# sqliteai/sqlite-vector

Hardware: AMD Instinct MI355X
Metric: vectors scanned/sec, L2 top-20 over Nx384 f32 (higher is better)
Workload: dtype f32; 1 GPU; 10Mx384 f32 L2 top-20 single-query; rows_per_gpu=10000000, dim=384, k=20, backend=HIP gfx950 x1

## Files before the change

include/vectorgpu_diag.h:

```cpp
#ifndef VECTORGPU_DIAG_H
#define VECTORGPU_DIAG_H

#include "vectorgpu.h"

#ifdef __cplusplus
extern "C" {
#endif

int vg_set_profiling(vg_corpus *c, int enabled);
int vg_last_kernel_ms(vg_corpus *c, float *scan_ms, float *merge_ms);
int vg_profile_mean_ms(vg_corpus *c, int *n_launches, float *scan_ms, float *merge_ms);
int vg_profile_mean_ms_ex(vg_corpus *c, int *n_launches, float *scan_ms, float *merge_ms, float *prepass_ms);
int vg_plan_scan_shape(int vtype, int dim, int metric, int *lanes_per_row, int *chunks_per_lane, int *long_rows);
int vg_batch_h_plan(long long stride_bytes, int k, int nq, int *waves, int *blocks_per_cu);
const char *vg_scan_kernel_name(vg_corpus *c, int metric);
int vg_filter_exact_evals(vg_corpus *c, unsigned long long *out_evals);
int vg_filter_guard_cooldown(vg_corpus *c);
int vg_batch_filter_exact_evals(vg_corpus *c, unsigned long long *out_evals);
void vg_reload_switches(void);
int vg_batch_last_path(const vg_corpus *c);
int vg_batch_q8_status(const vg_corpus *c);
int vg_batch_masked_plan(const vg_corpus *c, int metric, int *out_queries_per_pass, int *out_lpr, int *out_u);

int vg_corpus_pass_ms(const vg_corpus *c, int which, float *out_ms, long long *out_rows);
long long vg_stat_rows_appended(void);

int vg_shards_gather_stats(vg_shards *s, unsigned long long *out2);
int vg_shards_threaded(const vg_shards *s);
int vg_corpus_tie_stats(const vg_corpus *c, unsigned long long *out4);
int vg_shards_tie_stats(const vg_shards *s, unsigned long long *out4);
int vg_corpus_device_bytes(const vg_corpus *c, long long *out3);
int vg_shards_device_bytes(const vg_shards *s, long long *out3);
int vg_scan_distances_resident(vg_corpus *c, int metric, const void *query);
int vg_resident_distances_fetch(vg_corpus *c, int64_t pos0, int64_t n, float *out_host);
int vg_resident_distances_below(vg_corpus *c, int64_t pos0, float bound, uint64_t *out_pairs, int64_t cap, int64_t *out_count);

int vg_within_set_initial_capacity(vg_corpus *c, int64_t keys);
int vg_within_last_launches(const vg_corpus *c);
int vg_shards_within_set_initial_capacity(vg_shards *s, int64_t keys);
int vg_shards_within_last_launches(const vg_shards *s);

int vg_reference_topk_replay(const float *dist, int64_t n, int k, int64_t below_cap, int64_t *out_pos, double *out_dist);
int vg_reference_topk_replay_slabs(const float *dist, int64_t n, int k, int64_t slab_rows, int64_t below_cap, int64_t *out_pos, double *out_dist);


#ifdef __cplusplus
// ... 4 lines not shown
```

sqlite-vector_amd/__init__.py:

```python
import ctypes as C
import os

import numpy as np

HERE = os.path.dirname(os.path.abspath(__file__))
LIB_PATH = os.environ.get("VG_LIB_PATH") or os.path.join(HERE, "libvectorgpu.so")
EXT_PATH = os.path.join(HERE, "vector.so")

F32, F16, BF16, U8, I8 = 1, 2, 3, 4, 5
L2, SQUARED_L2, COSINE, DOT, L1 = 1, 2, 3, 4, 5
QUANT_U8, QUANT_S8 = 1, 2
TIE_POSITION, TIE_REFERENCE = 0, 1
KEY_EMPTY = 0xFFFFFFFFFFFFFFFF
HALF_TYPES = True
TYPE_SIZE = {F32: 4, F16: 2, BF16: 2, U8: 1, I8: 1}


class VectorGpuError(RuntimeError):
    pass


_lib = None


# ... 48 lines not shown
        "vg_scan_topk_keys": (i32, [vp, i32, vp, i32, vp, C.POINTER(i32)]),
        "vg_scan_topk_enqueue": (i32, [vp, i32, vp, i32]),
        "vg_scan_topk_collect": (i32, [vp, vp]),
        "vg_scan_topk_batch_keys": (i32, [vp, i32, vp, i32, i32, vp, vp]),
        "vg_shards_create": (i32, [vp, i32, i32, i32, i64, C.POINTER(vp)]),
        "vg_shards_destroy": (None, [vp]),
        "vg_shards_clear": (i32, [vp]),
        "vg_shards_count": (i32, [vp]),
        "vg_shards_rows": (i64, [vp]),
        "vg_shards_shard": (vp, [vp, i32]),
        "vg_shards_reserve": (i32, [vp, i64]),
        "vg_shards_set_rowid_base": (i32, [vp, i64]),
        "vg_shards_append": (i32, [vp, vp, i64, i64, vp]),
        "vg_shards_append_records": (i32, [vp, vp, i64]),
        "vg_shards_rowid_at": (i64, [vp, i64]),
        "vg_shards_scan_topk": (i32, [vp, i32, vp, i32, vp, vp, C.POINTER(i32)]),
        "vg_shards_scan_topk_batch": (i32, [vp, i32, vp, i32, i32, vp, vp, vp]),
        "vg_shards_scan_distances": (i32, [vp, i32, vp, vp]),
        "vg_shards_minmax": (i32, [vp, C.POINTER(C.c_float), C.POINTER(C.c_float), C.POINTER(i32)]),
        "vg_shards_quantize_rows": (i32, [vp, C.c_float, C.c_float, i32, i64, i64, vp]),
        "vg_merge_keys_batch": (i32, [vp, i32, i32, i32, vp, i32, vp, vp, vp]),
        "vg_scan_distances": (i32, [vp, i32, vp, vp]),
        "vg_scan_distances_device": (i32, [vp, i32, vp, vp, vp]),
        "vg_corpus_rowid_at": (i64, [vp, i64]),
        "vg_scan_topk_batch": (i32, [vp, i32, vp, i32, i32, vp, vp, vp]),
        "vg_quantize_query": (i32, [i32, vp, i32, C.c_float, C.c_float, i32, vp]),
        "vg_corpus_minmax": (i32, [vp, C.POINTER(C.c_float), C.POINTER(C.c_float), C.POINTER(i32)]),
        "vg_corpus_quantize_rows": (i32, [vp, C.c_float, C.c_float, i32, i64, i64, vp]),
        "vg_set_profiling": (i32, [vp, i32]),
        "vg_last_kernel_ms": (i32, [vp, C.POINTER(C.c_float), C.POINTER(C.c_float)]),
        "vg_profile_mean_ms": (i32, [vp, C.POINTER(i32), C.POINTER(C.c_float), C.POINTER(C.c_float)]),
        "vg_scan_kernel_name": (C.c_char_p, [vp, i32]),
        "vg_plan_scan_shape": (i32, [i32, i32, i32, C.POINTER(i32), C.POINTER(i32), C.POINTER(i32)]),
        "vg_batch_h_plan": (i32, [i64, i32, i32, C.POINTER(i32), C.POINTER(i32)]),
        "vg_profile_mean_ms_ex": (i32, [vp, C.POINTER(i32), C.POINTER(C.c_float), C.POINTER(C.c_float), C.POINTER(C.c_float)]),
        "vg_corpus_find_rowid": (i64, [vp, i64]),
        "vg_corpus_patch_rows": (i32, [vp, vp, i64, vp, i64]),
        "vg_corpus_delete_rows": (i32, [vp, vp, i64]),
        "vg_shards_find_rowid": (i64, [vp, i64]),
        "vg_shards_patch_rows": (i32, [vp, vp, i64, vp, i64]),
        "vg_shards_delete_rows": (i32, [vp, vp, i64]),
        "vg_filter_exact_evals": (i32, [vp, C.POINTER(C.c_ulonglong)]),
        "vg_filter_guard_cooldown": (i32, [vp]),
        "vg_batch_filter_exact_evals": (i32, [vp, C.POINTER(C.c_ulonglong)]),
        "vg_reload_switches": (None, []),
        "vg_batch_last_path": (i32, [vp]),
        "vg_batch_q8_status": (i32, [vp]),
        "vg_corpus_set_scan_filter": (i32, [vp, i32]),
        "vg_corpus_set_tie_order": (i32, [vp, i32]),
        "vg_corpus_tie_order": (i32, [vp]),
        "vg_corpus_tie_stats": (i32, [vp, vp]),
        "vg_corpus_pass_ms": (i32, [vp, i32, C.POINTER(C.c_float), C.POINTER(C.c_longlong)]),
        "vg_shards_set_tie_order": (i32, [vp, i32]),
        "vg_shards_set_scan_filter": (i32, [vp, i32]),
        "vg_shards_set_gather": (i32, [vp, i32]),
        "vg_shards_gather_stats": (i32, [vp, vp]),
        "vg_shards_tie_stats": (i32, [vp, vp]),
        "vg_shards_threaded": (i32, [vp]),
        "vg_slab_scan_begin": (i32, [i32, i32, i32, i32, vp, i32, i32, i64, i64, vp]),
        "vg_slab_scan_rows": (i32, [vp, vp, i64, i64, vp]),
        "vg_slab_scan_records": (i32, [vp, vp, i64]),
        "vg_slab_scan_finish": (i32, [vp, vp, vp, vp]),
        "vg_slab_scan_all": (i32, [vp, vp, vp, vp]),
        "vg_slab_scan_destroy": (None, [vp]),
        "vg_device_memory": (i32, [i32, vp, vp]),
        "vg_host_alloc": (i32, [C.c_size_t, C.POINTER(C.c_void_p)]),
# ... 135 lines not shown
        rows = np.ascontiguousarray(rows)
        assert rows.ndim == 2 and rows.shape[1] * rows.itemsize >= self.dim * TYPE_SIZE[self.vtype]
        ids = None if rowids is None else np.ascontiguousarray(rowids, dtype=np.int64)
        _check(lib().vg_corpus_append(self.h, _ptr(rows), rows.shape[0], rows.strides[0], _ptr(ids)))

    def append_strided(self, buf, n_rows, stride, rowids=None):
        buf = np.ascontiguousarray(buf)
        ids = None if rowids is None else np.ascontiguousarray(rowids, dtype=np.int64)
        _check(lib().vg_corpus_append(self.h, _ptr(buf), n_rows, stride, _ptr(ids)))

    def append_records(self, records, n):
        records = np.ascontiguousarray(records)
        _check(lib().vg_corpus_append_records(self.h, _ptr(records), n))

    def append_device(self, dev_ptr, n_rows, stride, rowids=None):
        ids = None if rowids is None else np.ascontiguousarray(rowids, dtype=np.int64)
        _check(lib().vg_corpus_append_device(self.h, C.c_void_p(dev_ptr), n_rows, stride, _ptr(ids)))

    def set_rowid_base(self, base):
        _check(lib().vg_corpus_set_rowid_base(self.h, base))

    def scan_topk(self, metric, query, k):
        query = np.ascontiguousarray(query)
        ids = np.zeros(max(k, 1), dtype=np.int64)
        dist = np.zeros(max(k, 1), dtype=np.float64)
        cnt = C.c_int(0)
        _check(lib().vg_scan_topk(self.h, metric, _ptr(query), k, _ptr(ids), _ptr(dist), C.byref(cnt)))
        return ids[:cnt.value], dist[:cnt.value]

    def scan_topk_device(self, metric, dev_query_ptr, k, dev_keys_ptr, stream=None):
        _check(lib().vg_scan_topk_device(self.h, metric, C.c_void_p(dev_query_ptr), k, C.c_void_p(dev_keys_ptr),
                                         C.c_void_p(stream) if stream else None))

    def scan_distances(self, metric, query):
        query = np.ascontiguousarray(query)
        out = np.empty(self.rows, dtype=np.float32)
        _check(lib().vg_scan_distances(self.h, metric, _ptr(query), _ptr(out)))
        return out

    def scan_within(self, metric, query, radius, limit=None):
        query = np.ascontiguousarray(query)
        m, held = C.c_int64(0), C.c_int64(0)
        _check(lib().vg_scan_within(self.h, metric, _ptr(query), float(radius), 0 if limit is None else max(int(limit), 0), C.byref(m), C.byref(held)))
        n = 0 if (limit is not None and limit <= 0) else held.value
        ids, dist = np.zeros(n, dtype=np.int64), np.zeros(n, dtype=np.float64)
        if n:
            _check(lib().vg_scan_within_fetch(self.h, 0, n, _ptr(ids), _ptr(dist)))
        return ids, dist, m.value

    def set_mask(self, bits=None, positions=None, rowids=None):
        return _set_mask(self, "vg_corpus", self.rows, bits, positions, rowids)

    def clear_mask(self):
        _check(lib().vg_corpus_clear_mask(self.h))

    def mask_count(self):
        return int(lib().vg_corpus_mask_count(self.h))

    def scan_topk_masked(self, metric, query, k):
        query = np.ascontiguousarray(query)
        ids = np.zeros(max(k, 1), dtype=np.int64)
        dist = np.zeros(max(k, 1), dtype=np.float64)
        cnt = C.c_int(0)
        _check(lib().vg_scan_topk_masked(self.h, metric, _ptr(query), k, _ptr(ids), _ptr(dist), C.byref(cnt)))
        return ids[:cnt.value], dist[:cnt.value]

# ... 392 lines not shown
```

sqlite-vector_amd/csrc/vg_api.hip:

```cpp
#include "vg_internal.h"

#include "vg_scan.h"


typedef void (*scan_fn_t)(ScanArgs);
scan_fn_t vg_pick_scan_kernel_ex(int vtype, int acc, int U);

typedef VgShape Shape;

static const int kAllowedU[] = {1, 2, 3, 4, 6, 8};

static int max_chunks_per_lane(int vtype, int acc, bool bf16_l2_u3) {
    if (vtype == VG_TYPE_F16) return 6;
    if (vtype == VG_TYPE_BF16) return (acc == A_L2 && !bf16_l2_u3) ? 6 : 3;
    return 8;
}

struct ShapeEnv { bool f16_round3, pref_round1, bf16_l2_u3, int_short_round3, force_long; int lpr_log2, u; };
static ShapeEnv shape_env() {
    ShapeEnv e;
    e.f16_round3 = vg_sw(SW_VG_SHAPE_F16_ROUND3, 0) != 0;
    e.pref_round1 = vg_sw(SW_VG_SHAPE_PREF_ROUND1, 0) != 0;
    e.bf16_l2_u3 = vg_sw(SW_VG_SHAPE_BF16_L2_U3, 0) != 0;
    e.int_short_round3 = vg_sw(SW_VG_SHAPE_INT_SHORT_ROUND3, 0) != 0;
// ... 172 lines not shown



#define VG_MERGE_THREADS 1024
__global__ __launch_bounds__(VG_MERGE_THREADS) void vg_merge_kernel(const uint64_t *cand, int nlists, int k,
                                                                    uint64_t *out_keys, const unsigned long long *mirror_src,
                                                                    unsigned long long *mirror_dst) {
    __shared__ __attribute__((aligned(16))) uint8_t scratch[VG_SEL_SCRATCH_BYTES];
    if (mirror_dst && blockIdx.x == 0 && threadIdx.x < 3) mirror_dst[threadIdx.x] = mirror_src[threadIdx.x];
    vg_select_lists(cand + (long long)blockIdx.x * nlists * VG_WAVE, nlists, k, out_keys + (long long)blockIdx.x * VG_WAVE, scratch);
}

int vg_launch_merge(const uint64_t *dev_cand, int nlists, int k, uint64_t *dev_out_keys, int nq, hipStream_t stream) {
    hipLaunchKernelGGL(vg_merge_kernel, dim3((unsigned)nq), dim3(VG_MERGE_THREADS), 0, stream, dev_cand, nlists, k, dev_out_keys,
                       (const unsigned long long *)nullptr, (unsigned long long *)nullptr);
    return (int)hipGetLastError();
}

static int launch_scan(vg_corpus *c, int metric, const uint8_t *dev_query, int k, uint64_t *dev_out_keys,
                       float *dev_out_dist, hipStream_t stream, const ScanPlan &plan = ScanPlan());

int vg_launch_plain_scan(vg_corpus *c, int metric, const uint8_t *dev_query, int k, uint64_t *dev_out_keys, hipStream_t stream,
                         const ScanPlan &plan) {
    return launch_scan(c, metric, dev_query, k, dev_out_keys, nullptr, stream, plan);
}
int vg_launch_merge_one(const uint64_t *dev_cand, int nlists, int k, uint64_t *dev_out_keys, hipStream_t stream,
                        const unsigned long long *mirror_src, unsigned long long *mirror_dst) {
    hipLaunchKernelGGL(vg_merge_kernel, dim3(1), dim3(VG_MERGE_THREADS), 0, stream, dev_cand, nlists, k, dev_out_keys, mirror_src, mirror_dst);
    return (int)hipGetLastError();
}
int vg_plain_scan_shape(const vg_corpus *c, int metric, VgShape *out) {
    choose_shape(c->nch, c->vtype, vg_metric_to_acc(metric), out);
    return 0;
}
long long vg_plain_scan_blocks(const vg_corpus *c, int64_t n_rows, const VgShape &s) {
    const int rpb = VG_WAVE >> s.lpr_log2;
    const long long nbatch = (n_rows + rpb - 1) / rpb;
    const int bpc = std::max(1, std::min(8, vg_sw(SW_VG_BLOCKS_PER_CU, 1)));
    long long blocks = (nbatch + VG_WAVES_PER_BLOCK - 1) / VG_WAVES_PER_BLOCK;
    blocks = std::max<long long>(1, std::min<long long>(blocks, (long long)c->cu_count * bpc));
    blocks = std::min<long long>(blocks, VG_SEL_MAX_HEADS);
    blocks = std::min<long long>(blocks, std::max<long long>(32, nbatch / (2 * VG_WAVES_PER_BLOCK)));
    return blocks;
}

static int launch_scan(vg_corpus *c, int metric, const uint8_t *dev_query, int k, uint64_t *dev_out_keys,
                       float *dev_out_dist, hipStream_t stream, const ScanPlan &plan) {
    int acc = vg_metric_to_acc(metric);
    if (acc < 0) return vg_fail(VG_ERR_INVALID, "unknown distance metric %d", metric);
    const int64_t n_rows = (plan.n_rows >= 0) ? std::min<int64_t>(plan.n_rows, c->n_rows) : c->n_rows;
    if (plan.ref_emit) c->ref_prefix_rows = -1;
    Shape s;
    choose_shape(c->nch, c->vtype, acc, &s);
    const bool whole_prefix = plan.ref_emit && !dev_out_dist && plan.n_rows < 0 && k > 0 && k <= VG_MAX_FUSED_K && !s.long_rows &&
                              n_rows < VG_REF_EMIT_MIN_ROWS;
    if (!whole_prefix && plan.allow_filter && plan.n_rows < 0 && !dev_out_dist && k <= VG_MAX_FUSED_K) {
        int rcf = vg_launch_scan_filter(c, metric, dev_query, k, dev_out_keys, stream, plan.ref_emit, plan.final_out);
        if (rcf != -1) return rcf;
    }
    if (acc == A_COS && (c->vtype == VG_TYPE_F16 || c->vtype == VG_TYPE_BF16) && !s.long_rows && vg_sw(SW_VG_HALF_COSN, 1)) {
        int rcn = vg_ensure_row_norms(c);
        if (rcn != VG_OK) return rcn;
        acc = A_COSN;
        if (stream != c->stream) {
            if (!c->norm_ev) HIP_TRY(hipEventCreateWithFlags(&c->norm_ev, hipEventDisableTiming));
            HIP_TRY(hipEventRecord(c->norm_ev, c->stream));
// ... 7 lines not shown
    if (whole_prefix) {
        int rcb = vg_ensure_ref_buffers(c, n_rows);
        if (rcb != VG_OK) return rcb;
        store_prefix = c->d_ref_prefix;
        emit_reset = c->d_below;
        c->ref_prefix_rows = n_rows;
    }
    const bool prefix_pass = store_prefix && !dev_out_dist && !s.long_rows && k > 0;
    scan_fn_t fn = (emitting || prefix_pass) ? vg_pick_scan_kernel_ex(c->vtype, acc, s.U) : pick_kernel(c->vtype, acc, s, use_nt_loads(c, n_rows));
    if (!fn) return vg_fail(VG_ERR_UNSUPPORTED, "no scan kernel for type %s", type_tag(c->vtype));

    const long long blocks = vg_plain_scan_blocks(c, n_rows, s);

    ScanArgs a{};
    a.rows = c->d_rows;
    a.query = dev_query;
    a.cand = plan.lists_out ? plan.lists_out : c->d_cand;
    a.out_dist = dev_out_dist;
    a.n_rows = n_rows;
    a.stride = c->stride;
    a.nch = c->nch;
    a.lpr_log2 = s.lpr_log2;
    a.k = k;
    a.root = (metric == VG_DIST_L2) ? 1 : 0;
    a.dim = c->dim;
    a.row_nn = (acc == A_COSN) ? c->d_xnorm : nullptr;
    a.init_keys = nullptr;
    a.emit = nullptr;
    a.emit_cap = 0;
    a.emit_reset = emit_reset;
    a.order = scan_order_for(c, n_rows);
    if (prefix_pass) a.out_dist = store_prefix;
    else a.emit_reset = nullptr;
    size_t qbytes = (size_t)c->nch * 16;
    if (s.long_rows) {
        const size_t slice = (size_t)VG_WAVE * VG_LONG_U;
        qbytes = ((c->nch + slice - 1) / slice) * slice * 16;
    }
    size_t smem = std::max<size_t>(qbytes, (size_t)VG_PUBLISH_LDS_BYTES);
    a.store_lds_off = 0;
    if (dev_out_dist && !s.long_rows) {
        a.store_lds_off = (int)((qbytes + 255) / 256 * 256);
        smem = std::max<size_t>(smem, (size_t)a.store_lds_off + (size_t)VG_WAVES_PER_BLOCK * VG_STORE_FLOATS * sizeof(float));
    }

    if (c->append_pending && stream != c->stream) HIP_TRY(hipStreamWaitEvent(stream, c->append_ev, 0));

    hipEvent_t *evs = plan.record ? vg_prof_slot(c, (uint8_t)((dev_out_dist == nullptr ? VG_EVF_MERGE : 0) | (emitting ? VG_EVF_PREPASS : 0))) : nullptr;
    if (evs) hipEventRecord(evs[0], stream);
    if (emitting) {
        const int64_t P = vg_ref_prefix_for(n_rows);
        int rcb = vg_ensure_ref_buffers(c, P);
        if (rcb != VG_OK) return rcb;
        ScanPlan pre;
        pre.n_rows = P;
        pre.allow_filter = false;
        pre.record = false;
        pre.store_prefix = c->d_ref_prefix;
        pre.emit_reset = c->d_below;
        int rcp = launch_scan(c, metric, dev_query, k, dev_out_keys, nullptr, stream, pre);
        if (rcp != VG_OK) return rcp;
        a.init_keys = dev_out_keys;
        a.emit = c->d_below;
        a.emit_cap = VG_BELOW_CAP;
        c->ref_prefix_rows = P;
        if (evs) hipEventRecord(evs[1], stream);
    }
    if (smem > 64 * 1024)
        HIP_TRY(hipFuncSetAttribute(reinterpret_cast<const void *>(fn), hipFuncAttributeMaxDynamicSharedMemorySize, (int)smem));
    hipLaunchKernelGGL(fn, dim3((unsigned)blocks), dim3(VG_BLOCK), smem, stream, a);
    if (evs) hipEventRecord(evs[2], stream);
    if (plan.lists_out) {
        if (plan.n_lists_out) *plan.n_lists_out = (int)blocks;
    } else if (!dev_out_dist) {
        hipLaunchKernelGGL(vg_merge_kernel, dim3(1), dim3(VG_MERGE_THREADS), 0, stream,
                           (const uint64_t *)c->d_cand, (int)blocks, k, plan.final_out ? plan.final_out : dev_out_keys,
                           (const unsigned long long *)nullptr, (unsigned long long *)nullptr);
    }
    if (evs) hipEventRecord(evs[3], stream);
    HIP_TRY(hipGetLastError());
    return VG_OK;
}

static bool host_direct(const vg_corpus *c) {
    const int v = vg_sw(SW_VG_HOST_DIRECT, -1);
    if (v >= 0) return v != 0;
    return c->n_rows * c->stride <= (64ll << 20);
}

static void stage_query(vg_corpus *c, const void *query) {
    memset(c->h_query, 0, (size_t)c->stride);
    memcpy(c->h_query, query, (size_t)c->dim * c->es);
}

static void slot_times(vg_corpus *c, int slot, float *scan_ms, float *merge_ms, float *prepass_ms) {
    hipEvent_t *evs = &c->ev[(size_t)slot * VG_PROF_EVS];
    const uint8_t fl = c->ev_flags[(size_t)slot];
    hipEventSynchronize(evs[3]);
    *scan_ms = 0.f; *merge_ms = 0.f; *prepass_ms = 0.f;
    if (fl & VG_EVF_PREPASS) hipEventElapsedTime(prepass_ms, evs[0], evs[1]);
    hipEventElapsedTime(scan_ms, evs[(fl & VG_EVF_PREPASS) ? 1 : 0], evs[2]);
    if (fl & VG_EVF_MERGE) hipEventElapsedTime(merge_ms, evs[2], evs[3]);
}

void vg_collect_timing(vg_corpus *c) {
    if (!c->profiling || c->prof_launches == 0) return;
    slot_times(c, (int)((c->prof_launches - 1) % VG_PROF_RING), &c->last_scan_ms, &c->last_merge_ms, &c->last_prepass_ms);
}

extern "C" float vg_key_distance(uint64_t key) { return vg_sortable_f32((uint32_t)(key >> 32)); }
extern "C" uint32_t vg_key_position(uint64_t key) { return (uint32_t)(key & 0xFFFFFFFFull); }

extern "C" int vg_scan_topk_device(vg_corpus *c, int metric, const void *dev_query, int k, uint64_t *dev_out_keys,
                                   void *stream) {
    if (!c || !dev_query || !dev_out_keys) return vg_fail(VG_ERR_INVALID, "vg_scan_topk_device: NULL argument");
    if (k < 1 || k > VG_MAX_FUSED_K) return vg_fail(VG_ERR_UNSUPPORTED, "vg_scan_topk_device: k must be in 1..%d", VG_MAX_FUSED_K);
    HIP_TRY(hipSetDevice(c->device));
    hipStream_t st = stream ? (hipStream_t)stream : c->stream;
    if (c->n_rows == 0) {
        HIP_TRY(hipMemsetAsync(dev_out_keys, 0xFF, VG_WAVE * sizeof(uint64_t), st));
        return VG_OK;
    }
    return launch_scan(c, metric, (const uint8_t *)dev_query, k, dev_out_keys, nullptr, st);
}

extern "C" int vg_scan_distances_device(vg_corpus *c, int metric, const void *dev_query, float *dev_out_dist, void *stream) {
    if (!c || !dev_query || !dev_out_dist) return vg_fail(VG_ERR_INVALID, "vg_scan_distances_device: NULL argument");
    HIP_TRY(hipSetDevice(c->device));
    if (c->n_rows == 0) return VG_OK;
    return launch_scan(c, metric, (const uint8_t *)dev_query, 0, nullptr, dev_out_dist, stream ? (hipStream_t)stream : c->stream);
}
// ... 279 lines not shown
```

sqlite-vector_amd/csrc/vg_corpus.hip:

```cpp
#include "vg_internal.h"

#include <atomic>
#include <mutex>
#include <utility>
#include <vector>

#include "vg_device.h"


static thread_local std::string g_err;

int vg_fail(int code, const char *fmt, ...) {
    char buf[1024];
    va_list ap;
    va_start(ap, fmt);
    vsnprintf(buf, sizeof(buf), fmt, ap);
    va_end(ap);
    g_err = buf;
    return code;
}

extern "C" const char *vg_last_error(void) { return g_err.c_str(); }
extern "C" void vg_set_last_error_(const char *msg) { g_err = msg ? msg : ""; }

// ... 36 lines not shown
    {"VG_BATCH_LONG_BPC", 1},
    {"VG_BATCH_MFMA", 0},
    {"VG_BATCH_MIN_QUERIES", 1},
    {"VG_BATCH_PREPASS", 1},
    {"VG_BATCH_Q8", 0},
    {"VG_BATCH_SLICE", 0},
    {"VG_BATCH_STAGES", 0},
    {"VG_BATCH_TILE_MAJOR", 0},
    {"VG_BLOCKS_PER_CU", 1},
    {"VG_F32_FILTER", 0},
    {"VG_FILTER_LPR_LOG2", 1},
    {"VG_FILTER_U", 1},
    {"VG_FORCE_LONG", 0},
    {"VG_HALF_COSN", 1},
    {"VG_HOST_DIRECT", 1},
    {"VG_KEYS_DIRECT", 1},
    {"VG_LPR_LOG2", 1},
    {"VG_MULTI_SCAN", 0},
    {"VG_NT", 1},
    {"VG_Q8_TWO_READS", 1},
    {"VG_RADIX_SELECT", 0},
    {"VG_REF_ALWAYS_EMIT", 1},
    {"VG_REF_STORE_MODE", 0},
    {"VG_SCAN_FILTER", 0},
    {"VG_SCAN_FILTER_MIN_MB", 0},
    {"VG_SCAN_FILTER_MIRROR_COPY", 1},
    {"VG_SCAN_FILTER_N4", 0},
    {"VG_SCAN_FILTER_NO_GUARD", 0},
    {"VG_SCAN_FILTER_PREMERGE", 1},
    {"VG_SCAN_FILTER_PREPASS", 1},
    {"VG_SCAN_FILTER_PREPASS_DIV", 1},
    {"VG_SCAN_FILTER_SHADOW", 0},
    {"VG_SCAN_ORDER", 1},
    {"VG_SHAPE_BF16_L2_U3", 1},
    {"VG_SHAPE_F16_ROUND3", 1},
    {"VG_SHAPE_INT_SHORT_ROUND3", 1},
    {"VG_SHAPE_PREF_ROUND1", 1},
    {"VG_U", 1},
};
std::atomic<int> vg_switch_values[VGSW_COUNT];
void vg_switches_read(void) {
    for (int i = 0; i < VGSW_COUNT; ++i) {
        int v = VGSW_UNSET;
#ifndef VG_LAB
        if (!vg_switch_names[i].lab)
#endif
        {
            const char *e = getenv(vg_switch_names[i].name);
            if (e && *e) {
                if (i == SW_VG_SCAN_FILTER_SHADOW) v = (unsigned char)e[0];
                else if (i == SW_VECTORGPU_SHARD_GATHER) v = (e[0] == 'r' || e[0] == 'R') ? 1 : 0;
                else v = atoi(e);
            }
        }
        vg_switch_values[i].store(v, std::memory_order_relaxed);
    }
}
__attribute__((constructor)) static void vg_switches_at_load(void) { vg_switches_read(); }
extern "C" void vg_reload_switches(void) { vg_switches_read(); }

extern "C" int vg_corpus_create(int device, int vtype, int dim, int64_t capacity_rows_hint, vg_corpus **out) {
    if (!out) return vg_fail(VG_ERR_INVALID, "vg_corpus_create: out is NULL");
    *out = nullptr;
    vg_switches_read();
    int es = vg_elem_size(vtype);
    if (es == 0) return vg_fail(VG_ERR_INVALID, "vg_corpus_create: unknown vector type %d", vtype);
    if (dim <= 0) return vg_fail(VG_ERR_INVALID, "vg_corpus_create: dimension must be positive (got %d)", dim);
    int ndev = vg_device_count();
    if (ndev <= 0) return vg_fail(VG_ERR_NO_DEVICE, "no HIP device available (the scan path is GPU-only)");
    if (device < 0 || device >= ndev) return vg_fail(VG_ERR_INVALID, "device %d out of range (0..%d)", device, ndev - 1);
    int64_t row_bytes = (int64_t)dim * es;
    if (row_bytes > 128 * 1024) return vg_fail(VG_ERR_UNSUPPORTED, "rows larger than 128 KiB are not supported (dim=%d): the query must fit the CU's 160 KiB LDS", dim);
    HIP_TRY(hipSetDevice(device));
    vg_corpus *c = new vg_corpus();
    c->device = device;
    c->vtype = vtype;
    c->dim = dim;
    c->es = es;
    c->nch = (int)((row_bytes + 15) / 16);
    c->stride = (int64_t)c->nch * 16;
    hipDeviceProp_t p;
    if (hipGetDeviceProperties(&p, device) != hipSuccess) { delete c; return vg_fail(VG_ERR_HIP, "hipGetDeviceProperties failed"); }
    c->cu_count = p.multiProcessorCount;
    c->max_blocks = c->cu_count * 8;
    hipError_t e;
    if ((e = hipStreamCreateWithFlags(&c->stream, hipStreamNonBlocking)) != hipSuccess ||
        (e = hipMalloc(&c->d_query, (size_t)c->stride)) != hipSuccess ||
        (e = hipHostMalloc(&c->h_query, (size_t)c->stride)) != hipSuccess ||
        (e = hipMalloc(&c->d_cand, (size_t)c->max_blocks * VG_WAVE * sizeof(uint64_t))) != hipSuccess ||
        (e = hipMalloc(&c->d_keys, VG_WAVE * sizeof(uint64_t))) != hipSuccess ||
        (e = hipHostMalloc(&c->h_keys, VG_WAVE * sizeof(uint64_t))) != hipSuccess) {
        vg_corpus_destroy(c);
        return vg_fail(VG_ERR_HIP, "vg_corpus_create: device setup failed: %s", hipGetErrorString(e));
    }
    if (capacity_rows_hint > 0) {
        e = hipMalloc(&c->d_rows, (size_t)(capacity_rows_hint * c->stride));
        if (e != hipSuccess) {
            vg_corpus_destroy(c);
            return vg_fail(VG_ERR_NOMEM, "vg_corpus_create: cannot allocate %lld bytes of HBM: %s",
                           (long long)(capacity_rows_hint * c->stride), hipGetErrorString(e));
        }
        c->cap_rows = capacity_rows_hint;
    }
    *out = c;
    return VG_OK;
}

extern "C" void vg_corpus_destroy(vg_corpus *c) {
    if (!c) return;
    hipSetDevice(c->device);
    if (c->stream) hipStreamSynchronize(c->stream);
    if (c->d_rows) hipFree(c->d_rows);
    if (c->d_query) hipFree(c->d_query);
    if (c->h_query) hipHostFree(c->h_query);
    if (c->d_cand) hipFree(c->d_cand);
    if (c->d_cand_pre) hipFree(c->d_cand_pre);
    if (c->d_keys) hipFree(c->d_keys);
    if (c->h_keys) hipHostFree(c->h_keys);
    if (c->d_dist) hipFree(c->d_dist);
    if (c->d_sel_keys) hipFree(c->d_sel_keys);
    if (c->d_sel_sorted) hipFree(c->d_sel_sorted);
    if (c->d_sel_temp) hipFree(c->d_sel_temp);
    for (int i = 0; i < 2; ++i) { if (c->pin[i]) hipHostFree(c->pin[i]); if (c->pin_ev[i]) hipEventDestroy(c->pin_ev[i]); }
    if (c->append_ev) hipEventDestroy(c->append_ev);
    if (c->d_stage) hipFree(c->d_stage);
    if (c->d_bq) hipFree(c->d_bq);
    if (c->h_bq) hipHostFree(c->h_bq);
// ... 677 lines not shown
```

sqlite-vector_amd/csrc/vg_device.h:

```cpp
#pragma once

#include <hip/hip_runtime.h>
#include <stdint.h>

#define VG_EMPTY_KEY 0xFFFFFFFFFFFFFFFFull
#define VG_WAVE 64
#define VG_BLOCK 1024
#define VG_WAVES_PER_BLOCK (VG_BLOCK / VG_WAVE)
#define VG_MAX_FUSED_K 64

enum { T_F32 = 1, T_F16 = 2, T_BF16 = 3, T_U8 = 4, T_I8 = 5 };
enum { M_L2 = 1, M_SQL2 = 2, M_COS = 3, M_DOT = 4, M_L1 = 5 };
enum { A_L2 = 0, A_COS = 1, A_DOT = 2, A_L1 = 3, A_COSN = 4  };

struct ScanArgs {
    const uint8_t *rows;
    const uint8_t *query;
    uint64_t *cand;
    float *out_dist;
    long long n_rows;
    long long stride;
    int nch;
    int lpr_log2;
    int k;
    int root;
    int dim;
    const float *row_nn;
    int store_lds_off;
    const uint64_t *init_keys;
    unsigned long long *emit;
    unsigned emit_cap;
    unsigned long long *emit_reset;
    int order;
    float within_r;
    unsigned long long within_cap;
    const uint64_t *mask;
};


__host__ __device__ inline uint32_t vg_f32_sortable(float d) {
    uint32_t b;
#if defined(__HIP_DEVICE_COMPILE__)
    b = __float_as_uint(d);
#else
    __builtin_memcpy(&b, &d, 4);
#endif
    return b ^ ((b >> 31) ? 0xFFFFFFFFu : 0x80000000u);
}
__host__ __device__ inline float vg_sortable_f32(uint32_t s) {
    uint32_t b = s ^ ((s >> 31) ? 0x80000000u : 0xFFFFFFFFu);
#if defined(__HIP_DEVICE_COMPILE__)
    return __uint_as_float(b);
#else
    float f; __builtin_memcpy(&f, &b, 4); return f;
#endif
}
__host__ __device__ inline uint64_t vg_make_key(float d, uint32_t pos) {
    return ((uint64_t)vg_f32_sortable(d) << 32) | (uint64_t)pos;
}


__device__ inline uint64_t vg_readlane64(uint64_t v, int lane_uniform) {
    uint32_t lo = (uint32_t)__builtin_amdgcn_readlane((int)(uint32_t)v, lane_uniform);
    uint32_t hi = (uint32_t)__builtin_amdgcn_readlane((int)(uint32_t)(v >> 32), lane_uniform);
    return ((uint64_t)hi << 32) | lo;
}

__device__ inline uint64_t vg_wave_shr1(uint64_t v) {
    const uint32_t lo = (uint32_t)__builtin_amdgcn_update_dpp(0, (int)(uint32_t)v, 0x138, 0xf, 0xf, false);
// ... 112 lines not shown
```

sqlite-vector_amd/csrc/vg_internal.h:

```cpp
#pragma once

#include "../../include/vectorgpu.h"
#include "../../include/vectorgpu_diag.h"

#include <hip/hip_runtime.h>

#include <algorithm>
#include <cmath>
#include <cstdarg>
#include <cstdio>
#include <cstdlib>
#include <cstring>
#include <string>
#include <vector>

#define VG_PROF_RING 1024
#define VG_PROF_EVS 4
#define VG_EVF_MERGE 1
#define VG_EVF_PREPASS 2
#define VG_WAVE_HOST 64

int vg_fail(int code, const char *fmt, ...);

#define HIP_TRY(expr)                                                                                     \
// ... 2 lines not shown
        if (e__ != hipSuccess)                                                                            \
            return vg_fail(e__ == hipErrorOutOfMemory ? VG_ERR_NOMEM : VG_ERR_HIP, "%s failed: %s (%s:%d)", \
                           #expr, hipGetErrorString(e__), __FILE__, __LINE__);                            \
    } while (0)


static inline int vg_elem_size(int vtype) {
    switch (vtype) {
        case VG_TYPE_F32: return 4;
        case VG_TYPE_F16: case VG_TYPE_BF16: return 2;
        case VG_TYPE_U8: case VG_TYPE_I8: return 1;
    }
    return 0;
}

struct vg_corpus {
    int device = 0;
    int vtype = 0;
    int dim = 0;
    int es = 0;
    int nch = 0;
    int64_t stride = 0;
    int64_t n_rows = 0;
    int64_t cap_rows = 0;
    uint8_t *d_rows = nullptr;
    std::vector<int64_t> rowids;
    bool rowids_ascending = true;
    int64_t rowid_base = 1;

    hipStream_t stream = nullptr;
    uint8_t *d_query = nullptr;
    uint8_t *h_query = nullptr;
    uint64_t *d_cand = nullptr;
    uint64_t *d_cand_pre = nullptr;
    uint64_t *d_keys = nullptr;
    uint64_t *h_keys = nullptr;
    float *d_dist = nullptr;
    int64_t d_dist_cap = 0;
    int64_t dist_valid_rows = 0;
    unsigned long long *d_below = nullptr;
    uint8_t *h_ref = nullptr;
    size_t h_ref_bytes = 0;
    std::vector<uint64_t> ref_pairs;
    int tie_order = 0;
    float *d_ref_prefix = nullptr;
    int64_t ref_prefix_cap = 0;
    int64_t ref_prefix_rows = -1;
    int ref_hot = 0;
    unsigned long long ref_stats[4] = {0, 0, 0, 0};
    uint64_t *d_sel_keys = nullptr, *d_sel_sorted = nullptr;
    void *d_sel_temp = nullptr;
    uint32_t *d_sel_state = nullptr;
    size_t sel_temp_bytes = 0;
    int64_t sel_cap = 0;
    uint8_t *pin[2] = {nullptr, nullptr};
    hipEvent_t pin_ev[2] = {nullptr, nullptr};
    bool pin_busy[2] = {false, false};
    int pin_idx = 0;
    uint8_t *d_stage = nullptr;
    hipEvent_t append_ev = nullptr;
    bool append_pending = false;
    bool enqueued = false;
    float *d_xnorm = nullptr;
    int64_t xnorm_rows = 0, xnorm_cap = 0;
    hipEvent_t norm_ev = nullptr;
    uint32_t *d_sx = nullptr;
// ... 147 lines not shown
```

sqlite-vector_amd/csrc/vg_scan.h:

```cpp
#pragma once

#include "vg_accum.h"
#include "vg_lists.h"

#define VG_PUBLISH_LDS_BYTES (VG_WAVES_PER_BLOCK * VG_WAVE * 8 + VG_SEL_SCRATCH_BYTES)

__device__ inline void vg_block_publish(uint8_t *smem, uint64_t mine, int k, uint64_t *dst) {
    const int lane = threadIdx.x & (VG_WAVE - 1);
    const int wave = threadIdx.x >> 6;
    uint64_t *lists = reinterpret_cast<uint64_t *>(smem);
    lists[wave * VG_WAVE + lane] = (lane < k) ? mine : VG_EMPTY_KEY;
    __syncthreads();
    vg_select_lists(lists, VG_WAVES_PER_BLOCK, k, dst, smem + VG_WAVES_PER_BLOCK * VG_WAVE * 8);
}

typedef uint32_t vg_u32x4 __attribute__((ext_vector_type(4)));

template <bool NT>
__device__ inline uint4 vg_load16(const uint8_t *p) {
    if (NT) {
        vg_u32x4 v = __builtin_nontemporal_load(reinterpret_cast<const vg_u32x4 *>(p));
        return make_uint4(v.x, v.y, v.z, v.w);
    }
    return *reinterpret_cast<const uint4 *>(p);
}

#ifndef VG_LOAD_PREDICATED
#define VG_LOAD_PREDICATED 0
#endif
static __device__ __attribute__((aligned(16))) uint32_t vg_zero_chunk[4] = {0u, 0u, 0u, 0u};

template <int U, bool NT>
__device__ inline void vg_load_batch(uint4 (&dst)[U], const uint8_t *rows, long long row, long long n_rows,
                                     long long stride, int sub, int lpr, int nch) {
    const uint8_t *p = rows + row * stride + (long long)sub * 16;
#pragma unroll
    for (int u = 0; u < U; ++u) {
        const int c = sub + u * lpr;
        if (VG_LOAD_PREDICATED) {
            uint4 v = make_uint4(0u, 0u, 0u, 0u);
            if (row < n_rows && c < nch) v = vg_load16<NT>(p + (long long)u * lpr * 16);
            dst[u] = v;
        } else {
            const uint8_t *src = (row < n_rows && c < nch) ? p + (long long)u * lpr * 16 : reinterpret_cast<const uint8_t *>(vg_zero_chunk);
            dst[u] = vg_load16<NT>(src);
        }
// ... 188 lines not shown
        for (int j = 0; j < NB - 1; ++j) load(buf[j], nn[j], b + j * wstride);
        while (b < b_end) {
#pragma unroll
            for (int j = 0; j < NB; ++j) {
                const long long bj = b + j * wstride;
                load(buf[(j + NB - 1) % NB], nn[(j + NB - 1) % NB], bj + (NB - 1) * wstride);
                if (bj < b_end) process(buf[j], nn[j], bj);
            }
            b += NB * wstride;
        }
    } else {
        load(buf[0], nn[0], b);
        while (b < b_end) {
            const long long bn = b + wstride;
            load(buf[1], nn[1], bn);
            process(buf[0], nn[0], b);
#pragma unroll
            for (int u = 0; u < U; ++u) buf[0][u] = buf[1][u];
            nn[0] = nn[1];
            b = bn;
        }
    }
    if constexpr (WITHIN) {
        if (wqueued > 0) vg_within_flush(wqueue, wqueued, a.emit, a.within_cap, lane);
        return;
    }
    if (store_mode) {
        for (int j = lane; j < in_line * rpb && line_row0 + j < a.n_rows; j += VG_WAVE) a.out_dist[line_row0 + j] = line[j];
        return;
    }

    __syncthreads();
    vg_block_publish(smem, mine, k, a.cand + (long long)blockIdx.x * VG_WAVE);
}

#define VG_LONG_U 2
template <int VT, int ACC, bool NT, bool WITHIN = false, bool MASKED = false>
__global__ __launch_bounds__(VG_BLOCK) void vg_scan_long_kernel(ScanArgs a) {
    extern __shared__ __attribute__((aligned(16))) uint8_t smem[];
    const int lane = threadIdx.x & (VG_WAVE - 1);
    const int wave = threadIdx.x >> 6;
    constexpr int U = VG_LONG_U;
    const int slice = VG_WAVE * U;
    const int S = (a.nch + slice - 1) / slice;
    const int nch_pad = S * slice;

    uint4 *qs = reinterpret_cast<uint4 *>(smem);
    for (int c = threadIdx.x; c < nch_pad; c += VG_BLOCK)
        qs[c] = (c < a.nch) ? reinterpret_cast<const uint4 *>(a.query)[c] : make_uint4(0u, 0u, 0u, 0u);
    __syncthreads();

    typename Accum<VT, ACC>::QStat qstat;
    {
        uint4 q0[U];
#pragma unroll
        for (int u = 0; u < U; ++u) q0[u] = qs[u * VG_WAVE + lane];
        qstat = Accum<VT, ACC>::template query_stat<U>(q0, 6);
        for (int s = 1; s < S; ++s) {
#pragma unroll
            for (int u = 0; u < U; ++u) q0[u] = qs[s * slice + u * VG_WAVE + lane];
            Accum<VT, ACC>::merge_qstat(qstat, Accum<VT, ACC>::template query_stat<U>(q0, 6));
        }
    }

    uint64_t mine = VG_EMPTY_KEY, thr = VG_EMPTY_KEY;
    const int k = a.k;
// ... 41 lines not shown
        if (ns == 0 && (!MASKED || m_cur)) {
            float d = acc.finish(qstat, 6, a.root);
            if constexpr (VT == T_F16 || VT == T_BF16) {
                if (acc.special(qstat, 6) && lane == 0)
                    d = vg_slow_distance<VT, ACC>(reinterpret_cast<const uint16_t *>(qs),
                                                  reinterpret_cast<const uint16_t *>(a.rows + row * a.stride), a.dim, a.root);
            }
            d = vg_clamp(d);
            if constexpr (WITHIN) {
                vg_within_offer(vg_make_key(d, (uint32_t)row), (lane == 0) && (d <= a.within_r) && (d < INFINITY), wqueue, wqueued, a.emit, a.within_cap, lane);
            } else if (store_mode) {
                if (lane == 0) a.out_dist[row] = d;
            } else {
                vg_list_offer(vg_make_key(d, (uint32_t)row), (lane == 0) && (d < INFINITY), mine, thr, lane, k);
            }
            acc.init();
        }
        if constexpr (MASKED) {
            if (ns == 0) { m_cur = m_nxt; m_nxt = vg_mask_bits(a.mask, nrow + wstride, 1, nrow + wstride < a.n_rows) != 0ull; }
        }
#pragma unroll
        for (int u = 0; u < U; ++u) cur[u] = nxt[u];
        row = nrow;
        s = ns;
    }
    if constexpr (WITHIN) {
        if (wqueued > 0) vg_within_flush(wqueue, wqueued, a.emit, a.within_cap, lane);
        return;
    }
    if (store_mode) return;

    __syncthreads();
    vg_block_publish(smem, mine, k, a.cand + (long long)blockIdx.x * VG_WAVE);
}


template <int VT>
__global__ __launch_bounds__(256) void vg_half_rownorm_kernel(const uint8_t *rows, long long row0, long long n, long long stride,
                                                              int nch, float *out) {
    const int sub = threadIdx.x & 15;
    const long long group = ((long long)blockIdx.x * blockDim.x + threadIdx.x) >> 4;
    const long long ngroups = ((long long)gridDim.x * blockDim.x) >> 4;
    for (long long r = group; r < n; r += ngroups) {
        const uint4 *p = reinterpret_cast<const uint4 *>(rows + (row0 + r) * stride);
        double s0 = 0.0, s1 = 0.0, s2 = 0.0, s3 = 0.0;
        for (int c = sub; c < nch; c += 16) {
            const uint4 v = p[c];
            const uint32_t w[4] = {v.x, v.y, v.z, v.w};
#pragma unroll
            for (int j = 0; j < 4; ++j) {
                float lo, hi;
                vg_unpack2<VT>(w[j], lo, hi);
                if (j & 1) { s2 += (double)(lo * lo); s3 += (double)(hi * hi); }
                else { s0 += (double)(lo * lo); s1 += (double)(hi * hi); }
            }
        }
        const double s = vg_group_sum((s0 + s1) + (s2 + s3), 4);
        if (sub == 0) { const float f = (float)s; out[row0 + r] = (s > 0.0 && f == 0.0f) ? 1.401298464324817e-45f : f; }
    }
}
```

sqlite-vector_amd/csrc/vg_switches.h:

```cpp
#pragma once
#include <atomic>
#include <climits>

enum VgSwitch {
    SW_VECTORGPU_SHARD_GATHER,
    SW_VECTORGPU_SHARD_THREADS,
    SW_VG_BATCH_BPC,
    SW_VG_BATCH_H_SPLIT,
    SW_VG_BATCH_H_WAVES,
    SW_VG_BATCH_LONG,
    SW_VG_BATCH_LONG_BPC,
    SW_VG_BATCH_MFMA,
    SW_VG_BATCH_MIN_QUERIES,
    SW_VG_BATCH_PREPASS,
    SW_VG_BATCH_Q8,
    SW_VG_BATCH_SLICE,
    SW_VG_BATCH_STAGES,
    SW_VG_BATCH_TILE_MAJOR,
    SW_VG_BLOCKS_PER_CU,
    SW_VG_F32_FILTER,
    SW_VG_FILTER_LPR_LOG2,
    SW_VG_FILTER_U,
    SW_VG_FORCE_LONG,
    SW_VG_HALF_COSN,
    SW_VG_HOST_DIRECT,
    SW_VG_KEYS_DIRECT,
    SW_VG_LPR_LOG2,
    SW_VG_MULTI_SCAN,
    SW_VG_NT,
    SW_VG_Q8_TWO_READS,
    SW_VG_RADIX_SELECT,
    SW_VG_REF_ALWAYS_EMIT,
    SW_VG_REF_STORE_MODE,
    SW_VG_SCAN_FILTER,
    SW_VG_SCAN_FILTER_MIN_MB,
    SW_VG_SCAN_FILTER_MIRROR_COPY,
    SW_VG_SCAN_FILTER_N4,
    SW_VG_SCAN_FILTER_NO_GUARD,
    SW_VG_SCAN_FILTER_PREMERGE,
    SW_VG_SCAN_FILTER_PREPASS,
    SW_VG_SCAN_FILTER_PREPASS_DIV,
    SW_VG_SCAN_FILTER_SHADOW,
    SW_VG_SCAN_ORDER,
    SW_VG_SHAPE_BF16_L2_U3,
    SW_VG_SHAPE_F16_ROUND3,
    SW_VG_SHAPE_INT_SHORT_ROUND3,
    SW_VG_SHAPE_PREF_ROUND1,
    SW_VG_U,
    VGSW_COUNT
};
#define VGSW_UNSET INT_MIN
extern std::atomic<int> vg_switch_values[VGSW_COUNT];
void vg_switches_read(void);
static inline int vg_sw(VgSwitch id, int dflt) { const int v = vg_switch_values[id].load(std::memory_order_relaxed); return v == VGSW_UNSET ? dflt : v; }
static inline bool vg_sw_set(VgSwitch id) { return vg_switch_values[id].load(std::memory_order_relaxed) != VGSW_UNSET; }
```

Before: 4.425 billion vectors/s.

## Fuse final top-k merge into scan kernel via last-block arrival counter

Adds a device arrival counter so that the last scan block to finish runs the cross-block top-k selection itself and writes the final keys. This removes the separate single-block merge kernel launch and the launch gap that precedes it. The cost is a release/acquire fence plus an atomic per block, and the final merge now runs serialized inside the scan kernel's tail. Profiling events and the candidate buffer allocation are adjusted to match, and a switch lets the path be turned off.

```diff
diff --git a/include/vectorgpu_diag.h b/include/vectorgpu_diag.h
--- a/include/vectorgpu_diag.h
+++ b/include/vectorgpu_diag.h
@@ -12,6 +12,7 @@
 int vg_profile_mean_ms(vg_corpus *c, int *n_launches, float *scan_ms, float *merge_ms);
 int vg_profile_mean_ms_ex(vg_corpus *c, int *n_launches, float *scan_ms, float *merge_ms, float *prepass_ms);
 int vg_plan_scan_shape(int vtype, int dim, int metric, int *lanes_per_row, int *chunks_per_lane, int *long_rows);
+int vg_scan_last_launch(const vg_corpus *c, int *out_blocks, int *out_tail_select);
 int vg_batch_h_plan(long long stride_bytes, int k, int nq, int *waves, int *blocks_per_cu);
 const char *vg_scan_kernel_name(vg_corpus *c, int metric);
 int vg_filter_exact_evals(vg_corpus *c, unsigned long long *out_evals);
diff --git a/sqlite-vector_amd/__init__.py b/sqlite-vector_amd/__init__.py
--- a/sqlite-vector_amd/__init__.py
+++ b/sqlite-vector_amd/__init__.py
@@ -104,6 +104,7 @@
         "vg_profile_mean_ms": (i32, [vp, C.POINTER(i32), C.POINTER(C.c_float), C.POINTER(C.c_float)]),
         "vg_scan_kernel_name": (C.c_char_p, [vp, i32]),
         "vg_plan_scan_shape": (i32, [i32, i32, i32, C.POINTER(i32), C.POINTER(i32), C.POINTER(i32)]),
+        "vg_scan_last_launch": (i32, [vp, C.POINTER(i32), C.POINTER(i32)]),
         "vg_batch_h_plan": (i32, [i64, i32, i32, C.POINTER(i32), C.POINTER(i32)]),
         "vg_profile_mean_ms_ex": (i32, [vp, C.POINTER(i32), C.POINTER(C.c_float), C.POINTER(C.c_float), C.POINTER(C.c_float)]),
         "vg_corpus_find_rowid": (i64, [vp, i64]),
@@ -305,6 +306,11 @@
         _check(lib().vg_scan_topk_device(self.h, metric, C.c_void_p(dev_query_ptr), k, C.c_void_p(dev_keys_ptr),
                                          C.c_void_p(stream) if stream else None))
 
+    def last_scan_launch(self):
+        blocks, tail = C.c_int(0), C.c_int(0)
+        _check(lib().vg_scan_last_launch(self.h, C.byref(blocks), C.byref(tail)))
+        return blocks.value, tail.value
+
     def scan_distances(self, metric, query):
         query = np.ascontiguousarray(query)
         out = np.empty(self.rows, dtype=np.float32)
diff --git a/sqlite-vector_amd/csrc/vg_api.hip b/sqlite-vector_amd/csrc/vg_api.hip
--- a/sqlite-vector_amd/csrc/vg_api.hip
+++ b/sqlite-vector_amd/csrc/vg_api.hip
@@ -228,6 +228,12 @@
 int vg_plain_scan_shape(const vg_corpus *c, int metric, VgShape *out) {
     choose_shape(c->nch, c->vtype, vg_metric_to_acc(metric), out);
     return 0;
+}
+extern "C" int vg_scan_last_launch(const vg_corpus *c, int *out_blocks, int *out_tail_select) {
+    if (!c) return vg_fail(VG_ERR_INVALID, "corpus is NULL");
+    if (out_blocks) *out_blocks = c->last_scan_blocks;
+    if (out_tail_select) *out_tail_select = c->last_scan_tail;
+    return VG_OK;
 }
 long long vg_plain_scan_blocks(const vg_corpus *c, int64_t n_rows, const VgShape &s) {
     const int rpb = VG_WAVE >> s.lpr_log2;
@@ -301,6 +307,13 @@
     a.order = scan_order_for(c, n_rows);
     if (prefix_pass) a.out_dist = store_prefix;
     else a.emit_reset = nullptr;
+    const bool tail = !dev_out_dist && !plan.lists_out && !emitting && !prefix_pass && k >= 1 && c->d_arrive &&
+                      (s.long_rows || vg_tail_fits(c->vtype, acc, s.U)) && vg_sw(SW_VG_SCAN_TAIL_SELECT, 1) != 0;
+    if (tail) {
+        a.final_out = plan.final_out ? plan.final_out : dev_out_keys;
+        a.arrive = c->d_arrive;
+    }
+    if (!dev_out_dist && !plan.lists_out && plan.record) { c->last_scan_blocks = (int)blocks; c->last_scan_tail = tail ? 1 : 0; }
     size_t qbytes = (size_t)c->nch * 16;
     if (s.long_rows) {
         const size_t slice = (size_t)VG_WAVE * VG_LONG_U;
@@ -315,7 +328,7 @@
 
     if (c->append_pending && stream != c->stream) HIP_TRY(hipStreamWaitEvent(stream, c->append_ev, 0));
 
-    hipEvent_t *evs = plan.record ? vg_prof_slot(c, (uint8_t)((dev_out_dist == nullptr ? VG_EVF_MERGE : 0) | (emitting ? VG_EVF_PREPASS : 0))) : nullptr;
+    hipEvent_t *evs = plan.record ? vg_prof_slot(c, (uint8_t)(((dev_out_dist == nullptr && !tail) ? VG_EVF_MERGE : 0) | (emitting ? VG_EVF_PREPASS : 0))) : nullptr;
     if (evs) hipEventRecord(evs[0], stream);
     if (emitting) {
         const int64_t P = vg_ref_prefix_for(n_rows);
@@ -341,12 +354,12 @@
     if (evs) hipEventRecord(evs[2], stream);
     if (plan.lists_out) {
         if (plan.n_lists_out) *plan.n_lists_out = (int)blocks;
-    } else if (!dev_out_dist) {
+    } else if (!dev_out_dist && !tail) {
         hipLaunchKernelGGL(vg_merge_kernel, dim3(1), dim3(VG_MERGE_THREADS), 0, stream,
                            (const uint64_t *)c->d_cand, (int)blocks, k, plan.final_out ? plan.final_out : dev_out_keys,
                            (const unsigned long long *)nullptr, (unsigned long long *)nullptr);
     }
-    if (evs) hipEventRecord(evs[3], stream);
+    if (evs && !tail) hipEventRecord(evs[3], stream);
     HIP_TRY(hipGetLastError());
     return VG_OK;
 }
@@ -365,7 +378,7 @@
 static void slot_times(vg_corpus *c, int slot, float *scan_ms, float *merge_ms, float *prepass_ms) {
     hipEvent_t *evs = &c->ev[(size_t)slot * VG_PROF_EVS];
     const uint8_t fl = c->ev_flags[(size_t)slot];
-    hipEventSynchronize(evs[3]);
+    hipEventSynchronize(evs[(fl & VG_EVF_MERGE) ? 3 : 2]);
     *scan_ms = 0.f; *merge_ms = 0.f; *prepass_ms = 0.f;
     if (fl & VG_EVF_PREPASS) hipEventElapsedTime(prepass_ms, evs[0], evs[1]);
     hipEventElapsedTime(scan_ms, evs[(fl & VG_EVF_PREPASS) ? 1 : 0], evs[2]);
diff --git a/sqlite-vector_amd/csrc/vg_corpus.hip b/sqlite-vector_amd/csrc/vg_corpus.hip
--- a/sqlite-vector_amd/csrc/vg_corpus.hip
+++ b/sqlite-vector_amd/csrc/vg_corpus.hip
@@ -92,6 +92,7 @@
     {"VG_SCAN_FILTER_PREPASS_DIV", 1},
     {"VG_SCAN_FILTER_SHADOW", 0},
     {"VG_SCAN_ORDER", 1},
+    {"VG_SCAN_TAIL_SELECT", 0},
     {"VG_SHAPE_BF16_L2_U3", 1},
     {"VG_SHAPE_F16_ROUND3", 1},
     {"VG_SHAPE_INT_SHORT_ROUND3", 1},
@@ -147,12 +148,14 @@
     if ((e = hipStreamCreateWithFlags(&c->stream, hipStreamNonBlocking)) != hipSuccess ||
         (e = hipMalloc(&c->d_query, (size_t)c->stride)) != hipSuccess ||
         (e = hipHostMalloc(&c->h_query, (size_t)c->stride)) != hipSuccess ||
-        (e = hipMalloc(&c->d_cand, (size_t)c->max_blocks * VG_WAVE * sizeof(uint64_t))) != hipSuccess ||
+        (e = hipMalloc(&c->d_cand, (size_t)c->max_blocks * VG_WAVE * sizeof(uint64_t) + 64)) != hipSuccess ||
+        (e = hipMemset(c->d_cand + (size_t)c->max_blocks * VG_WAVE, 0, 64)) != hipSuccess ||
         (e = hipMalloc(&c->d_keys, VG_WAVE * sizeof(uint64_t))) != hipSuccess ||
         (e = hipHostMalloc(&c->h_keys, VG_WAVE * sizeof(uint64_t))) != hipSuccess) {
         vg_corpus_destroy(c);
         return vg_fail(VG_ERR_HIP, "vg_corpus_create: device setup failed: %s", hipGetErrorString(e));
     }
+    c->d_arrive = reinterpret_cast<uint32_t *>(c->d_cand + (size_t)c->max_blocks * VG_WAVE);
     if (capacity_rows_hint > 0) {
         e = hipMalloc(&c->d_rows, (size_t)(capacity_rows_hint * c->stride));
         if (e != hipSuccess) {
diff --git a/sqlite-vector_amd/csrc/vg_device.h b/sqlite-vector_amd/csrc/vg_device.h
--- a/sqlite-vector_amd/csrc/vg_device.h
+++ b/sqlite-vector_amd/csrc/vg_device.h
@@ -35,6 +35,8 @@
     float within_r;
     unsigned long long within_cap;
     const uint64_t *mask;
+    uint64_t *final_out;
+    uint32_t *arrive;
 };
 
 
diff --git a/sqlite-vector_amd/csrc/vg_internal.h b/sqlite-vector_amd/csrc/vg_internal.h
--- a/sqlite-vector_amd/csrc/vg_internal.h
+++ b/sqlite-vector_amd/csrc/vg_internal.h
@@ -58,6 +58,9 @@
     uint8_t *d_query = nullptr;
     uint8_t *h_query = nullptr;
     uint64_t *d_cand = nullptr;
+    uint32_t *d_arrive = nullptr;
+    int last_scan_blocks = 0;
+    int last_scan_tail = 0;
     uint64_t *d_cand_pre = nullptr;
     uint64_t *d_keys = nullptr;
     uint64_t *h_keys = nullptr;
diff --git a/sqlite-vector_amd/csrc/vg_scan.h b/sqlite-vector_amd/csrc/vg_scan.h
--- a/sqlite-vector_amd/csrc/vg_scan.h
+++ b/sqlite-vector_amd/csrc/vg_scan.h
@@ -12,6 +12,30 @@
     lists[wave * VG_WAVE + lane] = (lane < k) ? mine : VG_EMPTY_KEY;
     __syncthreads();
     vg_select_lists(lists, VG_WAVES_PER_BLOCK, k, dst, smem + VG_WAVES_PER_BLOCK * VG_WAVE * 8);
+}
+
+__host__ __device__ constexpr bool vg_tail_fits(int vt, int acc, int U) {
+    return !((vt == T_F16 && acc == A_COS && U == 6) || (vt == T_BF16 && (acc == A_COS || acc == A_COSN) && U == 8) ||
+             (vt == T_BF16 && acc == A_DOT && U >= 6));
+}
+__device__ inline void vg_tail_select(uint8_t *smem, const ScanArgs &a, int k) {
+    asm volatile("s_waitcnt vmcnt(0)" ::: "memory");
+    __syncthreads();
+    unsigned int *ticket = reinterpret_cast<unsigned int *>(smem);
+    if (threadIdx.x == 0) {
+        __builtin_amdgcn_fence(__ATOMIC_RELEASE, "agent");
+        asm volatile("s_waitcnt vmcnt(0)" ::: "memory");
+        *ticket = __hip_atomic_fetch_add(a.arrive, 1u, __ATOMIC_RELAXED, __HIP_MEMORY_SCOPE_AGENT);
+    }
+    __syncthreads();
+    if (*ticket != gridDim.x - 1) return;
+    if (threadIdx.x == 0) {
+        __builtin_amdgcn_fence(__ATOMIC_ACQUIRE, "agent");
+        asm volatile("s_waitcnt vmcnt(0)" ::: "memory");
+    }
+    __syncthreads();
+    vg_select_lists(a.cand, (int)gridDim.x, k, a.final_out, smem + VG_WAVES_PER_BLOCK * VG_WAVE * 8);
+    if (threadIdx.x == 0) __hip_atomic_store(a.arrive, 0u, __ATOMIC_RELAXED, __HIP_MEMORY_SCOPE_AGENT);
 }
 
 typedef uint32_t vg_u32x4 __attribute__((ext_vector_type(4)));
@@ -266,6 +290,9 @@
 
     __syncthreads();
     vg_block_publish(smem, mine, k, a.cand + (long long)blockIdx.x * VG_WAVE);
+    if constexpr (!EX && !MASKED && vg_tail_fits(VT, ACC, U)) {
+        if (a.arrive) vg_tail_select(smem, a, k);
+    }
 }
 
 #define VG_LONG_U 2
@@ -373,6 +400,9 @@
 
     __syncthreads();
     vg_block_publish(smem, mine, k, a.cand + (long long)blockIdx.x * VG_WAVE);
+    if constexpr (!MASKED) {
+        if (a.arrive) vg_tail_select(smem, a, k);
+    }
 }
 
 
diff --git a/sqlite-vector_amd/csrc/vg_switches.h b/sqlite-vector_amd/csrc/vg_switches.h
--- a/sqlite-vector_amd/csrc/vg_switches.h
+++ b/sqlite-vector_amd/csrc/vg_switches.h
@@ -42,6 +42,7 @@
     SW_VG_SCAN_FILTER_PREPASS_DIV,
     SW_VG_SCAN_FILTER_SHADOW,
     SW_VG_SCAN_ORDER,
+    SW_VG_SCAN_TAIL_SELECT,
     SW_VG_SHAPE_BF16_L2_U3,
     SW_VG_SHAPE_F16_ROUND3,
     SW_VG_SHAPE_INT_SHORT_ROUND3,
```

New measurement: 4.419 billion vectors/s. About the same (-0.1%).
